# nyu-systems/CLM-GS

Hardware: AMD Instinct MI355X
Metric: training images/s (Rubble-4K 28M Gaussians clm_offload) (higher is better)
Workload: dtype f32

## Files before the change

### clm_gs_amd/csrc/isect3.hip

```cpp
#include <stdlib.h>

#include "common.h"
#include "gs_math.h"
#include "isect_math.h"
#include "radix.h"

namespace clmgs {

constexpr int I3_ROUNDS = 4;
constexpr int I3_CHUNK = 256 * I3_ROUNDS;
constexpr int I3_BIG = 64;
constexpr int I3_SCAN_BLOCKS = 64;

__host__ __device__ static inline int i3_chunks(int V) { return (V + I3_CHUNK - 1) / I3_CHUNK; }

struct RowBox { int x0, y0, bw, nt; unsigned long long mask; };

__device__ __forceinline__ RowBox unpack_row(unsigned long long b, unsigned long long m) {
  RowBox r;
  r.x0 = (int)(b & 0xFFFF); r.y0 = (int)((b >> 16) & 0xFFFF);
  const int x1 = (int)((b >> 32) & 0xFFFF), y1 = (int)(b >> 48);
  r.bw = x1 - r.x0; r.nt = r.bw * (y1 - r.y0);
  r.mask = r.nt > 64 ? ~0ull : (m & (r.nt == 64 ? ~0ull : ((1ull << r.nt) - 1ull)));
  return r;
}

constexpr int I3_WIN = 4096;

struct I3Window { int x0, y0, w, h; bool lds; };

__device__ __forceinline__ I3Window block_window(int x0, int y0, int x1, int y1, int* red ) {
  int v0 = x0, v1 = y0, v2 = -x1, v3 = -y1;
#pragma unroll
  for (int o = 32; o > 0; o >>= 1) {
    v0 = min(v0, __shfl_xor(v0, o, 64)); v1 = min(v1, __shfl_xor(v1, o, 64));
    v2 = min(v2, __shfl_xor(v2, o, 64)); v3 = min(v3, __shfl_xor(v3, o, 64));
  }
  const int wid = threadIdx.x >> 6;
  __syncthreads();
  if ((threadIdx.x & 63) == 0) { red[wid * 4 + 0] = v0; red[wid * 4 + 1] = v1; red[wid * 4 + 2] = v2; red[wid * 4 + 3] = v3; }
  __syncthreads();
  I3Window W;
  W.x0 = min(min(red[0], red[4]), min(red[8], red[12]));
  W.y0 = min(min(red[1], red[5]), min(red[9], red[13]));
  const int X1 = -min(min(red[2], red[6]), min(red[10], red[14]));
  const int Y1 = -min(min(red[3], red[7]), min(red[11], red[15]));
  W.w = max(X1 - W.x0, 0); W.h = max(Y1 - W.y0, 0);
  W.lds = (long long)W.w * W.h <= I3_WIN;
  return W;
}

__global__ void __launch_bounds__(256)
isect3_rows_kernel(int V, const int32_t* __restrict__ radii, const float* __restrict__ means2d,
                   const float4* __restrict__ packed, float tile_size, int tile_w, int tile_h,
                   unsigned long long* __restrict__ box_by_row, uint32_t* __restrict__ tile_cnt,
                   int64_t* __restrict__ row_cum, int64_t* __restrict__ blk_tot, int64_t* __restrict__ blk_ref) {
  __shared__ long long wsum[4];
  __shared__ int big_rows[I3_CHUNK];
  __shared__ int n_big;
  __shared__ unsigned long long rsum[4];
  __shared__ int red[16];
  __shared__ uint32_t win[I3_WIN];
  const int tid = threadIdx.x, chunk = blockIdx.x;
  if (tid == 0) n_big = 0;
  for (int q = tid; q < I3_WIN; q += 256) win[q] = 0u;
  __syncthreads();
  long long c[I3_ROUNDS];
  unsigned long long bx[I3_ROUNDS], mk[I3_ROUNDS];
  unsigned long long ref = 0ull;
  int wx0 = 1 << 30, wy0 = 1 << 30, wx1 = -(1 << 30), wy1 = -(1 << 30);
#pragma unroll
  for (int r = 0; r < I3_ROUNDS; ++r) {
    const int i = chunk * I3_CHUNK + r * 256 + tid;
    c[r] = 0; bx[r] = 0ull; mk[r] = 0ull;
    if (i < V) {
      const int rad = radii[i];
      unsigned long long b = 0ull, m = ~0ull;
      int cnt = 0;
      if (rad > 0) {
        const float2 mm = *reinterpret_cast<const float2*>(means2d + 2 * (size_t)i);
        const TileBox tb = tile_box(mm.x, mm.y, (float)rad, tile_size, tile_w, tile_h);
        b = pack_box(tb);
        if (packed) m = exact_tile_mask(packed + 4 * (size_t)i, tb.x0, tb.y0, tb.x1, tb.y1);
        const RowBox rb = unpack_row(b, m);
        ref += (unsigned long long)rb.nt;
        if (rb.nt > I3_BIG) {
          cnt = rb.nt;
          big_rows[atomicAdd(&n_big, 1)] = i;
        } else {
          cnt = __popcll(rb.mask);
          if (cnt) {
            bx[r] = b; mk[r] = rb.mask;
            wx0 = min(wx0, tb.x0); wy0 = min(wy0, tb.y0); wx1 = max(wx1, tb.x1); wy1 = max(wy1, tb.y1);
          }
        }
      }
      box_by_row[2 * (size_t)i] = cnt > 0 ? b : 0ull;
      box_by_row[2 * (size_t)i + 1] = m;
      c[r] = cnt;
    }
  }
  const I3Window W = block_window(wx0, wy0, wx1, wy1, red);
#pragma unroll
  for (int r = 0; r < I3_ROUNDS; ++r) {
    unsigned long long mm2 = mk[r];
    if (!mm2) continue;
    const RowBox rb = unpack_row(bx[r], mm2);
    while (mm2) {
      const int t = __ffsll((long long)mm2) - 1;
      mm2 &= mm2 - 1ull;
      const int ty = rb.y0 + t / rb.bw, tx = rb.x0 + t % rb.bw;
      if (W.lds) atomicAdd(&win[(ty - W.y0) * W.w + (tx - W.x0)], 1u);
      else atomicAdd(&tile_cnt[ty * tile_w + tx], 1u);
    }
  }
  {
    long long inc[I3_ROUNDS];
    long long carry = 0;
#pragma unroll
    for (int r = 0; r < I3_ROUNDS; ++r) {
      const long long incl = block_incl_scan_i64(c[r], wsum);
      inc[r] = carry + incl;
      carry += wsum[0] + wsum[1] + wsum[2] + wsum[3];
    }
    if (tid == 0) blk_tot[chunk] = carry;
#pragma unroll
    for (int r = 0; r < I3_ROUNDS; ++r) {
      const int i = chunk * I3_CHUNK + r * 256 + tid;
      if (i < V) row_cum[i] = inc[r];
    }
  }
  ref = (unsigned long long)wave_sum_i64((long long)ref);
  __syncthreads();
  if ((tid & 63) == 0) rsum[tid >> 6] = ref;
  if (W.lds) {
    const int nwin = W.w * W.h;
    for (int q = tid; q < nwin; q += 256) {
      const uint32_t v = win[q];
      if (v) atomicAdd(&tile_cnt[(W.y0 + q / W.w) * tile_w + W.x0 + q % W.w], v);
    }
  }
  __syncthreads();
  if (tid == 0) blk_ref[chunk] = (int64_t)(rsum[0] + rsum[1] + rsum[2] + rsum[3]);
  const int nb = n_big;
  for (int q = 0; q < nb; ++q) {
    const int i = big_rows[q];
    const RowBox rb = unpack_row(box_by_row[2 * (size_t)i], ~0ull);
    for (int t = tid; t < rb.nt; t += 256) {
      const int ty = t / rb.bw, tx = t - ty * rb.bw;
      atomicAdd(&tile_cnt[(rb.y0 + ty) * tile_w + rb.x0 + tx], 1u);
    }
  }
}

__global__ void __launch_bounds__(256)
isect3_rows_finish_kernel(int V, int64_t* __restrict__ row_cum, const int64_t* __restrict__ blk_tot,
                          const int64_t* __restrict__ blk_ref, int64_t* __restrict__ totals, int n_tiles,
                          const uint32_t* __restrict__ tile_cnt, int64_t* __restrict__ slice_tot) {
  __shared__ long long wsum[4];
  const int chunk = blockIdx.x, tid = threadIdx.x;
  for (int sl = chunk; sl < I3_SCAN_BLOCKS; sl += gridDim.x) {
    const int per = (n_tiles + I3_SCAN_BLOCKS - 1) / I3_SCAN_BLOCKS;
    const int t_lo = min(n_tiles, sl * per), t_hi = min(n_tiles, t_lo + per);
    long long sum = 0;
    for (int t = t_lo + tid; t < t_hi; t += 256) sum += tile_cnt[t];
    sum = wave_sum_i64(sum);
    __syncthreads();
    if ((tid & 63) == 0) wsum[tid >> 6] = sum;
    __syncthreads();
    if (tid == 0) slice_tot[sl] = wsum[0] + wsum[1] + wsum[2] + wsum[3];
    __syncthreads();
  }
  long long part = 0;
  for (int j = tid; j < chunk; j += 256) part += blk_tot[j];
  part = wave_sum_i64(part);
  if ((tid & 63) == 0) wsum[tid >> 6] = part;
  __syncthreads();
  const long long off = wsum[0] + wsum[1] + wsum[2] + wsum[3];
  if (chunk > 0) {
#pragma unroll
    for (int r = 0; r < I3_ROUNDS; ++r) {
      const int i = chunk * I3_CHUNK + r * 256 + tid;
      if (i < V) row_cum[i] += off;
    }
  }
  if (chunk == (int)gridDim.x - 1) {
    long long ref = 0;
    for (int j = tid; j < (int)gridDim.x; j += 256) ref += blk_ref[j];
    ref = wave_sum_i64(ref);
    __syncthreads();
    if ((tid & 63) == 0) wsum[tid >> 6] = ref;
    __syncthreads();
    if (tid == 0) { totals[0] = off + blk_tot[chunk]; totals[1] = wsum[0] + wsum[1] + wsum[2] + wsum[3]; }
  }
}

__global__ void __launch_bounds__(256)
isect3_tile_scan_kernel(int n_tiles, const uint32_t* __restrict__ tile_cnt, int64_t n, const int64_t* __restrict__ n_dev,
                        int32_t* __restrict__ offsets, uint32_t* __restrict__ cursor, uint32_t* __restrict__ big_count,
                        const int64_t* __restrict__ slice_tot) {
  __shared__ long long wsum[4];
  if (n_dev) n = min(n, *n_dev);
  const int tid = threadIdx.x;
  if (blockIdx.x == 0 && tid == 0) *big_count = 0u;
  const int per = (n_tiles + I3_SCAN_BLOCKS - 1) / I3_SCAN_BLOCKS;
  const int t_lo = min(n_tiles, (int)blockIdx.x * per), t_hi = min(n_tiles, t_lo + per);
  long long carry = 0;
  for (int sl = 0; sl < (int)blockIdx.x; ++sl) carry += slice_tot[sl];
  for (int base = t_lo; base < t_hi; base += 256) {
    const int t = base + tid;
    const uint32_t v = t < t_hi ? tile_cnt[t] : 0u;
    const long long incl = block_incl_scan_i64((long long)v, wsum);
    const long long ex = carry + incl - v;
    if (t < t_hi) {
      offsets[t] = (int32_t)min(ex, (long long)n);
      cursor[t] = (uint32_t)ex;
    }
    carry += wsum[0] + wsum[1] + wsum[2] + wsum[3];
    __syncthreads();
  }
}

struct I3Rec { uint32_t depth; int32_t row; int32_t slot; int32_t pad; };

__global__ void __launch_bounds__(256)
isect3_scatter_kernel(int V, const unsigned long long* __restrict__ box_by_row, const float* __restrict__ depths,
                      const int64_t* __restrict__ row_cum, int tile_w, uint32_t* __restrict__ cursor, int64_t n,
                      const int64_t* __restrict__ n_dev, int4* __restrict__ recs) {
  __shared__ int big_rows[I3_CHUNK];
  __shared__ int n_big;
  __shared__ int red[16];
  __shared__ uint32_t win[I3_WIN];
  if (n_dev) n = min(n, *n_dev);
  const int tid = threadIdx.x, chunk = blockIdx.x;
  if (tid == 0) n_big = 0;
  for (int q = tid; q < I3_WIN; q += 256) win[q] = 0u;
  __syncthreads();
  unsigned long long bx[I3_ROUNDS], mk[I3_ROUNDS];
  int wx0 = 1 << 30, wy0 = 1 << 30, wx1 = -(1 << 30), wy1 = -(1 << 30);
#pragma unroll
  for (int r = 0; r < I3_ROUNDS; ++r) {
    const int i = chunk * I3_CHUNK + r * 256 + tid;
    bx[r] = 0ull; mk[r] = 0ull;
    if (i >= V) continue;
    const unsigned long long b = box_by_row[2 * (size_t)i];
    if (b == 0ull) continue;
    const RowBox rb = unpack_row(b, box_by_row[2 * (size_t)i + 1]);
    if (rb.nt > I3_BIG) { big_rows[atomicAdd(&n_big, 1)] = i; continue; }
    bx[r] = b; mk[r] = rb.mask;
    wx0 = min(wx0, rb.x0); wy0 = min(wy0, rb.y0);
    wx1 = max(wx1, rb.x0 + rb.bw); wy1 = max(wy1, rb.y0 + rb.nt / rb.bw);
  }
  const I3Window W = block_window(wx0, wy0, wx1, wy1, red);
  if (W.lds) {
#pragma unroll
    for (int r = 0; r < I3_ROUNDS; ++r) {
      unsigned long long mm = mk[r];
      if (!mm) continue;
      const RowBox rb = unpack_row(bx[r], mm);
      while (mm) {
        const int t = __ffsll((long long)mm) - 1;
        mm &= mm - 1ull;
        atomicAdd(&win[(rb.y0 + t / rb.bw - W.y0) * W.w + (rb.x0 + t % rb.bw - W.x0)], 1u);
      }
    }
    __syncthreads();
    const int nwin = W.w * W.h;
    for (int q = tid; q < nwin; q += 256) {
      const uint32_t v = win[q];
      if (v) win[q] = atomicAdd(&cursor[(W.y0 + q / W.w) * tile_w + W.x0 + q % W.w], v);
    }
    __syncthreads();
  }
#pragma unroll
  for (int r = 0; r < I3_ROUNDS; ++r) {
    unsigned long long mm = mk[r];
    if (!mm) continue;
    const int i = chunk * I3_CHUNK + r * 256 + tid;
    const RowBox rb = unpack_row(bx[r], mm);
    const uint32_t dk = (uint32_t)__float_as_int(depths[i]);
    int slot = i > 0 ? (int)row_cum[i - 1] : 0;
    while (mm) {
      const int t = __ffsll((long long)mm) - 1;
      mm &= mm - 1ull;
      const int ty = rb.y0 + t / rb.bw, tx = rb.x0 + t % rb.bw;
      const uint32_t pos = W.lds ? atomicAdd(&win[(ty - W.y0) * W.w + (tx - W.x0)], 1u)
                                 : atomicAdd(&cursor[ty * tile_w + tx], 1u);
      if ((int64_t)pos < n) recs[pos] = make_int4((int)dk, i, slot, 0);
      ++slot;
    }
  }
  __syncthreads();
  const int nb = n_big;
  for (int q = 0; q < nb; ++q) {
    const int i = big_rows[q];
    const RowBox rb = unpack_row(box_by_row[2 * (size_t)i], ~0ull);
    const uint32_t dk = (uint32_t)__float_as_int(depths[i]);
    const int slot0 = i > 0 ? (int)row_cum[i - 1] : 0;
    for (int t = tid; t < rb.nt; t += 256) {
      const int ty = t / rb.bw, tx = t - ty * rb.bw;
      const uint32_t pos = atomicAdd(&cursor[(rb.y0 + ty) * tile_w + rb.x0 + tx], 1u);
      if ((int64_t)pos < n) recs[pos] = make_int4((int)dk, i, slot0 + t, 0);
    }
  }
}

template <int THREADS, typename SyncFn>
__device__ __forceinline__ void bitonic_sort_kv(unsigned long long* keys, int32_t* vals, int len, int tid, SyncFn sync) {
  int P = 1;
  while (P < len) P <<= 1;
  for (int k = 2; k <= P; k <<= 1) {
    for (int j = k >> 1; j > 0; j >>= 1) {
      sync();
      for (int c = tid; c < (P >> 1); c += THREADS) {
        const int lo = ((c & ~(j - 1)) << 1) | (c & (j - 1));
        const int hi = (j == (k >> 1)) ? (lo ^ (k - 1)) : (lo | j);
        if (hi < len) {
          const unsigned long long a = keys[lo], b = keys[hi];
          if (b < a) {
            keys[lo] = b; keys[hi] = a;
            const int32_t va = vals[lo], vb = vals[hi];
            vals[lo] = vb; vals[hi] = va;
          }
        }
      }
    }
  }
  sync();
}

constexpr int I3_SMALL = 1024;
constexpr int I3_LDS_BIG = 8192;

__device__ __forceinline__ void i3_write_out(int tile, int s, int len, const unsigned long long* keys, const int32_t* vals,
                                             int tid, int threads, int32_t* __restrict__ flatten_ids,
                                             int32_t* __restrict__ emit_slot, int64_t* __restrict__ isect_ids) {
  for (int q = tid; q < len; q += threads) {
    const unsigned long long k = keys[q];
    flatten_ids[s + q] = (int32_t)(k & 0xFFFFFFFFull);
    if (emit_slot) emit_slot[s + q] = vals[q];
    if (isect_ids) isect_ids[s + q] = ((int64_t)tile << 32) | (int64_t)(k >> 32);
  }
}

template <int LO, int CAP>
__global__ void __launch_bounds__(64)
isect3_sort_small_kernel(int n_tiles, const int32_t* __restrict__ offsets, int64_t n, const int64_t* __restrict__ n_dev,
                         const int4* __restrict__ recs, int32_t* __restrict__ flatten_ids,
                         int32_t* __restrict__ emit_slot, int64_t* __restrict__ isect_ids,
                         uint32_t* __restrict__ big_count, int32_t* __restrict__ big_list) {
  __shared__ unsigned long long keys[CAP];
  __shared__ int32_t vals[CAP];
  if (n_dev) n = min(n, *n_dev);
  const int tile = (int)xcd_remap(blockIdx.x, (unsigned)n_tiles);
  const int tid = threadIdx.x;
  const int s = offsets[tile];
  const int e = (tile == n_tiles - 1) ? (int)n : offsets[tile + 1];
  const int len = e - s;
  if (CAP == I3_SMALL && len > I3_SMALL && tid == 0) big_list[atomicAdd(big_count, 1u)] = tile;
  if (len <= LO || len > CAP) return;
  for (int q = tid; q < len; q += 64) {
    const int4 r = recs[s + q];
    keys[q] = ((unsigned long long)(uint32_t)r.x << 32) | (unsigned long long)(uint32_t)r.y;
    vals[q] = r.z;
  }
  bitonic_sort_kv<64>(keys, vals, len, tid, [] { __syncthreads(); });
  i3_write_out(tile, s, len, keys, vals, tid, 64, flatten_ids, emit_slot, isect_ids);
}

template <int E>
__device__ __forceinline__ void rank_sort_tile(unsigned long long* keys, int tile, int s, int len, int tid,
                                               const int4* __restrict__ recs, int32_t* __restrict__ flatten_ids,
                                               int32_t* __restrict__ emit_slot, int64_t* __restrict__ isect_ids) {
  unsigned long long key[E];
  int32_t slot[E];
#pragma unroll
  for (int r = 0; r < E; ++r) {
    const int q = tid + 64 * r;
    key[r] = ~0ull; slot[r] = 0;
    if (q < len) {
      const int4 rc = recs[s + q];
      key[r] = ((unsigned long long)(uint32_t)rc.x << 32) | (unsigned long long)(uint32_t)rc.y;
      slot[r] = rc.z;
      keys[q] = key[r];
    }
  }
  __syncthreads();
  int cnt[E];
#pragma unroll
  for (int r = 0; r < E; ++r) cnt[r] = 0;
  int j = 0;
  for (; j + 4 <= len; j += 4) {
    const unsigned long long k0 = keys[j], k1 = keys[j + 1], k2 = keys[j + 2], k3 = keys[j + 3];
#pragma unroll
    for (int r = 0; r < E; ++r)
      cnt[r] += (int)(k0 < key[r]) + (int)(k1 < key[r]) + (int)(k2 < key[r]) + (int)(k3 < key[r]);
  }
  for (; j < len; ++j) {
    const unsigned long long k0 = keys[j];
#pragma unroll
    for (int r = 0; r < E; ++r) cnt[r] += (int)(k0 < key[r]);
  }
#pragma unroll
  for (int r = 0; r < E; ++r) {
    if (tid + 64 * r < len) {
      const int o = s + cnt[r];
      flatten_ids[o] = (int32_t)(key[r] & 0xFFFFFFFFull);
      if (emit_slot) emit_slot[o] = slot[r];
      if (isect_ids) isect_ids[o] = ((int64_t)tile << 32) | (int64_t)(key[r] >> 32);
    }
  }
}

__global__ void __launch_bounds__(64)
isect3_sort_rank_kernel(int n_tiles, const int32_t* __restrict__ offsets, int64_t n, const int64_t* __restrict__ n_dev,
                        const int4* __restrict__ recs, int32_t* __restrict__ flatten_ids,
                        int32_t* __restrict__ emit_slot, int64_t* __restrict__ isect_ids) {
  constexpr int CAP = 256;
  __shared__ unsigned long long keys[CAP];
  if (n_dev) n = min(n, *n_dev);
  const int tile = (int)xcd_remap(blockIdx.x, (unsigned)n_tiles);
  const int tid = threadIdx.x;
  const int s = offsets[tile];
  const int e = (tile == n_tiles - 1) ? (int)n : offsets[tile + 1];
  const int len = e - s;
  if (len <= 0 || len > CAP) return;
  if (len <= 64) rank_sort_tile<1>(keys, tile, s, len, tid, recs, flatten_ids, emit_slot, isect_ids);
  else if (len <= 128) rank_sort_tile<2>(keys, tile, s, len, tid, recs, flatten_ids, emit_slot, isect_ids);
  else if (len <= 192) rank_sort_tile<3>(keys, tile, s, len, tid, recs, flatten_ids, emit_slot, isect_ids);
  else rank_sort_tile<4>(keys, tile, s, len, tid, recs, flatten_ids, emit_slot, isect_ids);
}

__global__ void __launch_bounds__(256)
isect3_sort_big_kernel(int n_tiles, const int32_t* __restrict__ offsets, int64_t n, const int64_t* __restrict__ n_dev,
                       const int4* __restrict__ recs, unsigned long long* __restrict__ gkeys, int32_t* __restrict__ gvals,
                       int32_t* __restrict__ flatten_ids, int32_t* __restrict__ emit_slot,
                       int64_t* __restrict__ isect_ids, const uint32_t* __restrict__ big_count,
                       const int32_t* __restrict__ big_list) {
  extern __shared__ __attribute__((aligned(16))) unsigned char dyn[];
  if (n_dev) n = min(n, *n_dev);
  const int tid = threadIdx.x;
  const int n_big = (int)*big_count;
  for (int w = blockIdx.x; w < n_big; w += gridDim.x) {
    const int tile = big_list[w];
    const int s = offsets[tile];
    const int e = (tile == n_tiles - 1) ? (int)n : offsets[tile + 1];
    const int len = e - s;
    __syncthreads();
    unsigned long long* keys;
    int32_t* vals;
    if (len <= I3_LDS_BIG) {
      keys = reinterpret_cast<unsigned long long*>(dyn);
      vals = reinterpret_cast<int32_t*>(dyn + sizeof(unsigned long long) * I3_LDS_BIG);
    } else {
      keys = gkeys + s;
      vals = gvals + s;
    }
    for (int q = tid; q < len; q += 256) {
      const int4 r = recs[s + q];
      keys[q] = ((unsigned long long)(uint32_t)r.x << 32) | (unsigned long long)(uint32_t)r.y;
      vals[q] = r.z;
    }
    bitonic_sort_kv<256>(keys, vals, len, tid, [] { __threadfence_block(); __syncthreads(); });
    i3_write_out(tile, s, len, keys, vals, tid, 256, flatten_ids, emit_slot, isect_ids);
  }
}

}

using namespace clmgs;

static inline size_t i3_front_layout(int V, int n_tiles, size_t* o_cnt, size_t* o_tot, size_t* o_ref) {
  size_t o = align_up((size_t)V * 16, 256);
  *o_cnt = o; o += align_up((size_t)n_tiles * 4, 256) + align_up((size_t)I3_SCAN_BLOCKS * 8, 256);
  *o_tot = o; o += align_up((size_t)i3_chunks(V) * 8, 256);
  *o_ref = o; o += align_up((size_t)i3_chunks(V) * 8, 256);
  return o + 256;
}

extern "C" size_t clmgs_isect3_front_temp_bytes(int V, int n_tiles) {
  if (V <= 0) return 256;
  size_t a, b, c;
  return i3_front_layout(V, n_tiles, &a, &b, &c);
}

extern "C" int clmgs_isect3_front(void* stream, int V, const float* means2d, const int32_t* radii, int tile_size,
                                  int tile_width, int tile_height, const void* packed, int64_t* totals,
                                  int64_t* row_cum, void* temp, size_t temp_bytes) {
  CLMGS_CHECK_ARG(V >= 0 && tile_size > 0 && tile_width > 0 && tile_height > 0);
  CLMGS_CHECK_ARG(tile_width < 65536 && tile_height < 65536 && (int64_t)tile_width * tile_height < ((int64_t)1 << 31));
  if (V == 0) return 0;
  const int n_tiles = tile_width * tile_height;
  CLMGS_CHECK_ARG(means2d && radii && totals && row_cum && temp);
  CLMGS_CHECK_ARG(!packed || tile_size == 16);
  CLMGS_CHECK_ARG(temp_bytes >= clmgs_isect3_front_temp_bytes(V, n_tiles));
  hipStream_t s = (hipStream_t)stream;
  size_t o_cnt, o_tot, o_ref;
  i3_front_layout(V, n_tiles, &o_cnt, &o_tot, &o_ref);
  char* base = (char*)temp;
  unsigned long long* box_by_row = (unsigned long long*)base;
  uint32_t* tile_cnt = (uint32_t*)(base + o_cnt);
  int64_t* blk_tot = (int64_t*)(base + o_tot);
  int64_t* blk_ref = (int64_t*)(base + o_ref);
  CLMGS_HIP(hipMemsetAsync(tile_cnt, 0, (size_t)n_tiles * 4, s));
  const int nck = i3_chunks(V);
  hipLaunchKernelGGL(isect3_rows_kernel, dim3(nck), dim3(256), 0, s, V, radii, means2d, (const float4*)packed,
                     (float)tile_size, tile_width, tile_height, box_by_row, tile_cnt, row_cum, blk_tot, blk_ref);
  int64_t* slice_tot = (int64_t*)(base + o_cnt + align_up((size_t)n_tiles * 4, 256));
  hipLaunchKernelGGL(isect3_rows_finish_kernel, dim3(nck), dim3(256), 0, s, V, row_cum, blk_tot, blk_ref, totals, n_tiles,
                     (const uint32_t*)tile_cnt, slice_tot);
  CLMGS_LAUNCH_CHECK();
  return 0;
}

static inline size_t i3_bin_layout(int64_t n, int n_tiles, size_t* o_cur, size_t* o_keys, size_t* o_vals) {
  size_t o = align_up((size_t)n * 16, 256);
  *o_cur = o; o += 2 * align_up((size_t)n_tiles * 4, 256) + 256;
  *o_keys = o; o += align_up((size_t)n * 8, 256);
  *o_vals = o; o += align_up((size_t)n * 4, 256);
  return o + 256;
}

extern "C" size_t clmgs_isect3_bin_temp_bytes(int64_t n_isects, int n_tiles) {
  if (n_isects <= 0) return 256;
  size_t a, b, c;
  return i3_bin_layout(n_isects, n_tiles, &a, &b, &c);
}

static int isect3_bin_impl(void* stream, int V, int64_t n_isects, const int64_t* n_dev, const float* depths,
                           int tile_width, int tile_height, const int64_t* row_cum, const void* front_temp,
                           int32_t* flatten_ids, int32_t* offsets, int64_t* isect_ids, int32_t* emit_slot, void* temp,
                           size_t temp_bytes) {
  CLMGS_CHECK_ARG(V >= 0 && n_isects >= 0 && offsets && tile_width > 0 && tile_height > 0);
  hipStream_t s = (hipStream_t)stream;
  const int n_tiles = tile_width * tile_height;
  if (n_isects == 0 || V == 0) {
    CLMGS_HIP(hipMemsetAsync(offsets, 0, sizeof(int32_t) * (size_t)n_tiles, s));
    return 0;
  }
  CLMGS_CHECK_ARG(n_isects < ((int64_t)1 << 31));
  CLMGS_CHECK_ARG(depths && row_cum && front_temp && flatten_ids && temp);
  CLMGS_CHECK_ARG(temp_bytes >= clmgs_isect3_bin_temp_bytes(n_isects, n_tiles));
  size_t f_cnt, f_tot, f_ref;
  i3_front_layout(V, n_tiles, &f_cnt, &f_tot, &f_ref);
  const unsigned long long* box_by_row = (const unsigned long long*)front_temp;
  const uint32_t* tile_cnt = (const uint32_t*)((const char*)front_temp + f_cnt);
  size_t o_cur, o_keys, o_vals;
  i3_bin_layout(n_isects, n_tiles, &o_cur, &o_keys, &o_vals);
  char* base = (char*)temp;
  int4* recs = (int4*)base;
  uint32_t* cursor = (uint32_t*)(base + o_cur);
  unsigned long long* gkeys = (unsigned long long*)(base + o_keys);
  int32_t* gvals = (int32_t*)(base + o_vals);
  int32_t* big_list = (int32_t*)(base + o_cur + align_up((size_t)n_tiles * 4, 256));
  uint32_t* big_count = (uint32_t*)(base + o_cur + 2 * align_up((size_t)n_tiles * 4, 256));
  const int64_t* slice_tot = (const int64_t*)((const char*)front_temp + f_cnt + align_up((size_t)n_tiles * 4, 256));
  hipLaunchKernelGGL(isect3_tile_scan_kernel, dim3(I3_SCAN_BLOCKS), dim3(256), 0, s, n_tiles, tile_cnt, n_isects, n_dev,
                     offsets, cursor, big_count, slice_tot);
  hipLaunchKernelGGL(isect3_scatter_kernel, dim3(i3_chunks(V)), dim3(256), 0, s, V, box_by_row, depths, row_cum,
                     tile_width, cursor, n_isects, n_dev, recs);
  hipLaunchKernelGGL(isect3_sort_rank_kernel, dim3(n_tiles), dim3(64), 0, s, n_tiles, (const int32_t*)offsets, n_isects,
                     n_dev, (const int4*)recs, flatten_ids, emit_slot, isect_ids);
  hipLaunchKernelGGL((isect3_sort_small_kernel<256, 512>), dim3(n_tiles), dim3(64), 0, s, n_tiles, (const int32_t*)offsets,
                     n_isects, n_dev, (const int4*)recs, flatten_ids, emit_slot, isect_ids, big_count, big_list);
  hipLaunchKernelGGL((isect3_sort_small_kernel<512, I3_SMALL>), dim3(n_tiles), dim3(64), 0, s, n_tiles,
                     (const int32_t*)offsets, n_isects, n_dev, (const int4*)recs, flatten_ids, emit_slot, isect_ids,
                     big_count, big_list);
  static bool lds_set = false;
  const size_t big_lds = (size_t)I3_LDS_BIG * 12;
  if (!lds_set) {
    CLMGS_HIP(hipFuncSetAttribute((const void*)isect3_sort_big_kernel, hipFuncAttributeMaxDynamicSharedMemorySize,
                                  (int)big_lds));
    lds_set = true;
  }
  hipLaunchKernelGGL(isect3_sort_big_kernel, dim3(min(n_tiles, 256)), dim3(256), big_lds, s, n_tiles,
                     (const int32_t*)offsets, n_isects, n_dev, (const int4*)recs, gkeys, gvals, flatten_ids, emit_slot,
                     isect_ids, (const uint32_t*)big_count, (const int32_t*)big_list);
  CLMGS_LAUNCH_CHECK();
  return 0;
}

extern "C" int clmgs_isect3_bin(void* stream, int V, int64_t n_isects, const float* depths, int tile_width,
                                int tile_height, const int64_t* row_cum, const void* front_temp, int32_t* flatten_ids,
                                int32_t* offsets, int64_t* isect_ids, int32_t* emit_slot, void* temp, size_t temp_bytes) {
  return isect3_bin_impl(stream, V, n_isects, nullptr, depths, tile_width, tile_height, row_cum, front_temp, flatten_ids,
                         offsets, isect_ids, emit_slot, temp, temp_bytes);
}

extern "C" int clmgs_isect3_bin_dev(void* stream, int V, int64_t capacity, const int64_t* n_isects_dev,
                                    const float* depths, int tile_width, int tile_height, const int64_t* row_cum,
                                    const void* front_temp, int32_t* flatten_ids, int32_t* offsets, int64_t* isect_ids,
                                    int32_t* emit_slot, void* temp, size_t temp_bytes) {
  CLMGS_CHECK_ARG(n_isects_dev && capacity > 0);
  return isect3_bin_impl(stream, V, capacity, n_isects_dev, depths, tile_width, tile_height, row_cum, front_temp,
                         flatten_ids, offsets, isect_ids, emit_slot, temp, temp_bytes);
}
```

Measured before the change: 206.2.

## Restructure tile-intersection pipeline into single-wave blocks with hierarchical scans and tile lists

Rewrites the intersection row, finish, tile-scan and scatter kernels to use 64-thread single-wave blocks. Block-level scans and window reductions become wave shuffles, and LDS windows are processed per group of four rows. Prefix offsets now use per-superchunk atomically accumulated totals, so each chunk no longer sums all earlier chunk totals. The rank sort kernel now builds per-size-class tile lists so that the medium and large sorts launch compact grids instead of one block per tile. The cost is more global atomics for group totals and big-row handling, and smaller LDS windows that may fall back to global atomics more often.

New measurement: 202.3. 1.9% lower.

```diff
diff --git a/clm_gs_amd/csrc/isect3.hip b/clm_gs_amd/csrc/isect3.hip
--- a/clm_gs_amd/csrc/isect3.hip
+++ b/clm_gs_amd/csrc/isect3.hip
@@ -7,10 +7,13 @@
 
 namespace clmgs {
 
-constexpr int I3_ROUNDS = 4;
-constexpr int I3_CHUNK = 256 * I3_ROUNDS;
+constexpr int I3_ROUNDS = 16;
+constexpr int I3_CHUNK = 64 * I3_ROUNDS;
+constexpr int I3_GROUP = 4;
 constexpr int I3_BIG = 64;
-constexpr int I3_SCAN_BLOCKS = 64;
+constexpr int I3_SCAN_BLOCKS = 256;
+constexpr int I3_SUPER = 64;
+constexpr int I3_LIST_GRID = 1024;
 
 __host__ __device__ static inline int i3_chunks(int V) { return (V + I3_CHUNK - 1) / I3_CHUNK; }
 
@@ -25,282 +28,262 @@
   return r;
 }
 
-constexpr int I3_WIN = 4096;
+constexpr int I3_WIN = 896;
 
 struct I3Window { int x0, y0, w, h; bool lds; };
 
-__device__ __forceinline__ I3Window block_window(int x0, int y0, int x1, int y1, int* red ) {
+__device__ __forceinline__ I3Window wave_window(int x0, int y0, int x1, int y1) {
   int v0 = x0, v1 = y0, v2 = -x1, v3 = -y1;
 #pragma unroll
   for (int o = 32; o > 0; o >>= 1) {
     v0 = min(v0, __shfl_xor(v0, o, 64)); v1 = min(v1, __shfl_xor(v1, o, 64));
     v2 = min(v2, __shfl_xor(v2, o, 64)); v3 = min(v3, __shfl_xor(v3, o, 64));
   }
-  const int wid = threadIdx.x >> 6;
-  __syncthreads();
-  if ((threadIdx.x & 63) == 0) { red[wid * 4 + 0] = v0; red[wid * 4 + 1] = v1; red[wid * 4 + 2] = v2; red[wid * 4 + 3] = v3; }
-  __syncthreads();
   I3Window W;
-  W.x0 = min(min(red[0], red[4]), min(red[8], red[12]));
-  W.y0 = min(min(red[1], red[5]), min(red[9], red[13]));
-  const int X1 = -min(min(red[2], red[6]), min(red[10], red[14]));
-  const int Y1 = -min(min(red[3], red[7]), min(red[11], red[15]));
-  W.w = max(X1 - W.x0, 0); W.h = max(Y1 - W.y0, 0);
+  W.x0 = v0; W.y0 = v1;
+  W.w = max(-v2 - v0, 0); W.h = max(-v3 - v1, 0);
   W.lds = (long long)W.w * W.h <= I3_WIN;
   return W;
 }
 
-__global__ void __launch_bounds__(256)
+__global__ void __launch_bounds__(64)
 isect3_rows_kernel(int V, const int32_t* __restrict__ radii, const float* __restrict__ means2d,
                    const float4* __restrict__ packed, float tile_size, int tile_w, int tile_h,
                    unsigned long long* __restrict__ box_by_row, uint32_t* __restrict__ tile_cnt,
-                   int64_t* __restrict__ row_cum, int64_t* __restrict__ blk_tot, int64_t* __restrict__ blk_ref) {
-  __shared__ long long wsum[4];
-  __shared__ int big_rows[I3_CHUNK];
-  __shared__ int n_big;
-  __shared__ unsigned long long rsum[4];
-  __shared__ int red[16];
+                   int64_t* __restrict__ row_cum, int64_t* __restrict__ blk_tot, unsigned long long* __restrict__ grp) {
   __shared__ uint32_t win[I3_WIN];
-  const int tid = threadIdx.x, chunk = blockIdx.x;
-  if (tid == 0) n_big = 0;
-  for (int q = tid; q < I3_WIN; q += 256) win[q] = 0u;
-  __syncthreads();
-  long long c[I3_ROUNDS];
-  unsigned long long bx[I3_ROUNDS], mk[I3_ROUNDS];
+  const int lane = threadIdx.x, chunk = blockIdx.x;
+  long long carry = 0;
   unsigned long long ref = 0ull;
-  int wx0 = 1 << 30, wy0 = 1 << 30, wx1 = -(1 << 30), wy1 = -(1 << 30);
-#pragma unroll
-  for (int r = 0; r < I3_ROUNDS; ++r) {
-    const int i = chunk * I3_CHUNK + r * 256 + tid;
-    c[r] = 0; bx[r] = 0ull; mk[r] = 0ull;
-    if (i < V) {
-      const int rad = radii[i];
-      unsigned long long b = 0ull, m = ~0ull;
-      int cnt = 0;
-      if (rad > 0) {
-        const float2 mm = *reinterpret_cast<const float2*>(means2d + 2 * (size_t)i);
-        const TileBox tb = tile_box(mm.x, mm.y, (float)rad, tile_size, tile_w, tile_h);
-        b = pack_box(tb);
-        if (packed) m = exact_tile_mask(packed + 4 * (size_t)i, tb.x0, tb.y0, tb.x1, tb.y1);
-        const RowBox rb = unpack_row(b, m);
-        ref += (unsigned long long)rb.nt;
-        if (rb.nt > I3_BIG) {
-          cnt = rb.nt;
-          big_rows[atomicAdd(&n_big, 1)] = i;
-        } else {
-          cnt = __popcll(rb.mask);
-          if (cnt) {
-            bx[r] = b; mk[r] = rb.mask;
-            wx0 = min(wx0, tb.x0); wy0 = min(wy0, tb.y0); wx1 = max(wx1, tb.x1); wy1 = max(wy1, tb.y1);
+  for (int g = 0; g < I3_ROUNDS / I3_GROUP; ++g) {
+    const int base = chunk * I3_CHUNK + g * I3_GROUP * 64;
+    if (base >= V) break;
+    unsigned long long bx[I3_GROUP], mk[I3_GROUP];
+    int wx0 = 1 << 30, wy0 = 1 << 30, wx1 = -(1 << 30), wy1 = -(1 << 30);
+#pragma unroll
+    for (int r = 0; r < I3_GROUP; ++r) {
+      const int i = base + r * 64 + lane;
+      bx[r] = 0ull; mk[r] = 0ull;
+      long long cnt = 0;
+      if (i < V) {
+        const int rad = radii[i];
+        unsigned long long b = 0ull, m = ~0ull;
+        if (rad > 0) {
+          const float2 mm = *reinterpret_cast<const float2*>(means2d + 2 * (size_t)i);
+          const TileBox tb = tile_box(mm.x, mm.y, (float)rad, tile_size, tile_w, tile_h);
+          b = pack_box(tb);
+          if (packed) m = exact_tile_mask(packed + 4 * (size_t)i, tb.x0, tb.y0, tb.x1, tb.y1);
+          const RowBox rb = unpack_row(b, m);
+          ref += (unsigned long long)rb.nt;
+          if (rb.nt > I3_BIG) {
+            cnt = rb.nt;
+            bx[r] = b; mk[r] = ~0ull;
+          } else {
+            cnt = __popcll(rb.mask);
+            if (cnt) {
+              bx[r] = b; mk[r] = rb.mask;
+              wx0 = min(wx0, tb.x0); wy0 = min(wy0, tb.y0); wx1 = max(wx1, tb.x1); wy1 = max(wy1, tb.y1);
+            }
           }
         }
-      }
-      box_by_row[2 * (size_t)i] = cnt > 0 ? b : 0ull;
-      box_by_row[2 * (size_t)i + 1] = m;
-      c[r] = cnt;
-    }
-  }
-  const I3Window W = block_window(wx0, wy0, wx1, wy1, red);
-#pragma unroll
-  for (int r = 0; r < I3_ROUNDS; ++r) {
-    unsigned long long mm2 = mk[r];
-    if (!mm2) continue;
-    const RowBox rb = unpack_row(bx[r], mm2);
-    while (mm2) {
-      const int t = __ffsll((long long)mm2) - 1;
-      mm2 &= mm2 - 1ull;
-      const int ty = rb.y0 + t / rb.bw, tx = rb.x0 + t % rb.bw;
-      if (W.lds) atomicAdd(&win[(ty - W.y0) * W.w + (tx - W.x0)], 1u);
-      else atomicAdd(&tile_cnt[ty * tile_w + tx], 1u);
-    }
-  }
-  {
-    long long inc[I3_ROUNDS];
-    long long carry = 0;
-#pragma unroll
-    for (int r = 0; r < I3_ROUNDS; ++r) {
-      const long long incl = block_incl_scan_i64(c[r], wsum);
-      inc[r] = carry + incl;
-      carry += wsum[0] + wsum[1] + wsum[2] + wsum[3];
-    }
-    if (tid == 0) blk_tot[chunk] = carry;
-#pragma unroll
-    for (int r = 0; r < I3_ROUNDS; ++r) {
-      const int i = chunk * I3_CHUNK + r * 256 + tid;
-      if (i < V) row_cum[i] = inc[r];
+        box_by_row[2 * (size_t)i] = cnt > 0 ? b : 0ull;
+        box_by_row[2 * (size_t)i + 1] = m;
+      }
+      const long long incl = wave_incl_scan_i64(cnt, lane);
+      if (i < V) row_cum[i] = carry + incl;
+      carry += __shfl(incl, 63, 64);
+    }
+    const I3Window W = wave_window(wx0, wy0, wx1, wy1);
+    const int nwin = W.w * W.h;
+    if (W.lds)
+      for (int q = lane; q < nwin; q += 64) win[q] = 0u;
+    __syncthreads();
+#pragma unroll
+    for (int r = 0; r < I3_GROUP; ++r) {
+      unsigned long long mm2 = mk[r];
+      const RowBox rb = unpack_row(bx[r], mm2);
+      if (rb.nt > I3_BIG) continue;
+      while (mm2) {
+        const int t = __ffsll((long long)mm2) - 1;
+        mm2 &= mm2 - 1ull;
+        const int ty = rb.y0 + t / rb.bw, tx = rb.x0 + t % rb.bw;
+        if (W.lds) atomicAdd(&win[(ty - W.y0) * W.w + (tx - W.x0)], 1u);
+        else atomicAdd(&tile_cnt[ty * tile_w + tx], 1u);
+      }
+    }
+    __syncthreads();
+    if (W.lds) {
+      for (int q = lane; q < nwin; q += 64) {
+        const uint32_t v = win[q];
+        if (v) atomicAdd(&tile_cnt[(W.y0 + q / W.w) * tile_w + W.x0 + q % W.w], v);
+      }
+    }
+    __syncthreads();
+#pragma unroll
+    for (int r = 0; r < I3_GROUP; ++r) {
+      unsigned long long bigs = __ballot(unpack_row(bx[r], mk[r]).nt > I3_BIG);
+      while (bigs) {
+        const int src = __ffsll((long long)bigs) - 1;
+        bigs &= bigs - 1ull;
+        const RowBox rb = unpack_row(__shfl(bx[r], src, 64), ~0ull);
+        for (int t = lane; t < rb.nt; t += 64) {
+          const int ty = t / rb.bw, tx = t - ty * rb.bw;
+          atomicAdd(&tile_cnt[(rb.y0 + ty) * tile_w + rb.x0 + tx], 1u);
+        }
+      }
     }
   }
   ref = (unsigned long long)wave_sum_i64((long long)ref);
-  __syncthreads();
-  if ((tid & 63) == 0) rsum[tid >> 6] = ref;
-  if (W.lds) {
-    const int nwin = W.w * W.h;
-    for (int q = tid; q < nwin; q += 256) {
-      const uint32_t v = win[q];
-      if (v) atomicAdd(&tile_cnt[(W.y0 + q / W.w) * tile_w + W.x0 + q % W.w], v);
-    }
-  }
-  __syncthreads();
-  if (tid == 0) blk_ref[chunk] = (int64_t)(rsum[0] + rsum[1] + rsum[2] + rsum[3]);
-  const int nb = n_big;
-  for (int q = 0; q < nb; ++q) {
-    const int i = big_rows[q];
-    const RowBox rb = unpack_row(box_by_row[2 * (size_t)i], ~0ull);
-    for (int t = tid; t < rb.nt; t += 256) {
-      const int ty = t / rb.bw, tx = t - ty * rb.bw;
-      atomicAdd(&tile_cnt[(rb.y0 + ty) * tile_w + rb.x0 + tx], 1u);
-    }
-  }
-}
-
-__global__ void __launch_bounds__(256)
+  if (lane == 0) {
+    blk_tot[chunk] = carry;
+    atomicAdd(&grp[2 * (chunk / I3_SUPER)], (unsigned long long)carry);
+    atomicAdd(&grp[2 * (chunk / I3_SUPER) + 1], ref);
+  }
+}
+
+__global__ void __launch_bounds__(64)
 isect3_rows_finish_kernel(int V, int64_t* __restrict__ row_cum, const int64_t* __restrict__ blk_tot,
-                          const int64_t* __restrict__ blk_ref, int64_t* __restrict__ totals, int n_tiles,
+                          const unsigned long long* __restrict__ grp, int64_t* __restrict__ totals, int n_tiles,
                           const uint32_t* __restrict__ tile_cnt, int64_t* __restrict__ slice_tot) {
-  __shared__ long long wsum[4];
-  const int chunk = blockIdx.x, tid = threadIdx.x;
+  const int chunk = blockIdx.x, lane = threadIdx.x;
   for (int sl = chunk; sl < I3_SCAN_BLOCKS; sl += gridDim.x) {
     const int per = (n_tiles + I3_SCAN_BLOCKS - 1) / I3_SCAN_BLOCKS;
     const int t_lo = min(n_tiles, sl * per), t_hi = min(n_tiles, t_lo + per);
     long long sum = 0;
-    for (int t = t_lo + tid; t < t_hi; t += 256) sum += tile_cnt[t];
+    for (int t = t_lo + lane; t < t_hi; t += 64) sum += tile_cnt[t];
     sum = wave_sum_i64(sum);
-    __syncthreads();
-    if ((tid & 63) == 0) wsum[tid >> 6] = sum;
-    __syncthreads();
-    if (tid == 0) slice_tot[sl] = wsum[0] + wsum[1] + wsum[2] + wsum[3];
-    __syncthreads();
-  }
+    if (lane == 0) slice_tot[sl] = sum;
+  }
+  const int g0 = chunk / I3_SUPER;
   long long part = 0;
-  for (int j = tid; j < chunk; j += 256) part += blk_tot[j];
-  part = wave_sum_i64(part);
-  if ((tid & 63) == 0) wsum[tid >> 6] = part;
-  __syncthreads();
-  const long long off = wsum[0] + wsum[1] + wsum[2] + wsum[3];
+  for (int j = lane; j < g0; j += 64) part += (long long)grp[2 * j];
+  if (g0 * I3_SUPER + lane < chunk) part += blk_tot[g0 * I3_SUPER + lane];
+  const long long off = wave_sum_i64(part);
   if (chunk > 0) {
-#pragma unroll
+#pragma unroll 4
     for (int r = 0; r < I3_ROUNDS; ++r) {
-      const int i = chunk * I3_CHUNK + r * 256 + tid;
+      const int i = chunk * I3_CHUNK + r * 64 + lane;
       if (i < V) row_cum[i] += off;
     }
   }
   if (chunk == (int)gridDim.x - 1) {
     long long ref = 0;
-    for (int j = tid; j < (int)gridDim.x; j += 256) ref += blk_ref[j];
+    for (int j = lane; j <= g0; j += 64) ref += (long long)grp[2 * j + 1];
     ref = wave_sum_i64(ref);
-    __syncthreads();
-    if ((tid & 63) == 0) wsum[tid >> 6] = ref;
-    __syncthreads();
-    if (tid == 0) { totals[0] = off + blk_tot[chunk]; totals[1] = wsum[0] + wsum[1] + wsum[2] + wsum[3]; }
-  }
-}
-
-__global__ void __launch_bounds__(256)
+    if (lane == 0) { totals[0] = off + blk_tot[chunk]; totals[1] = ref; }
+  }
+}
+
+__global__ void __launch_bounds__(64)
 isect3_tile_scan_kernel(int n_tiles, const uint32_t* __restrict__ tile_cnt, int64_t n, const int64_t* __restrict__ n_dev,
-                        int32_t* __restrict__ offsets, uint32_t* __restrict__ cursor, uint32_t* __restrict__ big_count,
+                        int32_t* __restrict__ offsets, uint32_t* __restrict__ cursor, uint32_t* __restrict__ list_count,
                         const int64_t* __restrict__ slice_tot) {
-  __shared__ long long wsum[4];
   if (n_dev) n = min(n, *n_dev);
-  const int tid = threadIdx.x;
-  if (blockIdx.x == 0 && tid == 0) *big_count = 0u;
+  const int lane = threadIdx.x;
+  if (blockIdx.x == 0 && lane < 3) list_count[lane] = 0u;
   const int per = (n_tiles + I3_SCAN_BLOCKS - 1) / I3_SCAN_BLOCKS;
   const int t_lo = min(n_tiles, (int)blockIdx.x * per), t_hi = min(n_tiles, t_lo + per);
-  long long carry = 0;
-  for (int sl = 0; sl < (int)blockIdx.x; ++sl) carry += slice_tot[sl];
-  for (int base = t_lo; base < t_hi; base += 256) {
-    const int t = base + tid;
+  long long part = 0;
+  for (int sl = lane; sl < (int)blockIdx.x; sl += 64) part += slice_tot[sl];
+  long long carry = wave_sum_i64(part);
+  for (int base = t_lo; base < t_hi; base += 64) {
+    const int t = base + lane;
     const uint32_t v = t < t_hi ? tile_cnt[t] : 0u;
-    const long long incl = block_incl_scan_i64((long long)v, wsum);
+    const long long incl = wave_incl_scan_i64((long long)v, lane);
     const long long ex = carry + incl - v;
     if (t < t_hi) {
       offsets[t] = (int32_t)min(ex, (long long)n);
       cursor[t] = (uint32_t)ex;
     }
-    carry += wsum[0] + wsum[1] + wsum[2] + wsum[3];
-    __syncthreads();
+    carry += __shfl(incl, 63, 64);
   }
 }
 
 struct I3Rec { uint32_t depth; int32_t row; int32_t slot; int32_t pad; };
 
-__global__ void __launch_bounds__(256)
+__global__ void __launch_bounds__(64)
 isect3_scatter_kernel(int V, const unsigned long long* __restrict__ box_by_row, const float* __restrict__ depths,
                       const int64_t* __restrict__ row_cum, int tile_w, uint32_t* __restrict__ cursor, int64_t n,
                       const int64_t* __restrict__ n_dev, int4* __restrict__ recs) {
-  __shared__ int big_rows[I3_CHUNK];
-  __shared__ int n_big;
-  __shared__ int red[16];
   __shared__ uint32_t win[I3_WIN];
   if (n_dev) n = min(n, *n_dev);
-  const int tid = threadIdx.x, chunk = blockIdx.x;
-  if (tid == 0) n_big = 0;
-  for (int q = tid; q < I3_WIN; q += 256) win[q] = 0u;
-  __syncthreads();
-  unsigned long long bx[I3_ROUNDS], mk[I3_ROUNDS];
-  int wx0 = 1 << 30, wy0 = 1 << 30, wx1 = -(1 << 30), wy1 = -(1 << 30);
-#pragma unroll
-  for (int r = 0; r < I3_ROUNDS; ++r) {
-    const int i = chunk * I3_CHUNK + r * 256 + tid;
-    bx[r] = 0ull; mk[r] = 0ull;
-    if (i >= V) continue;
-    const unsigned long long b = box_by_row[2 * (size_t)i];
-    if (b == 0ull) continue;
-    const RowBox rb = unpack_row(b, box_by_row[2 * (size_t)i + 1]);
-    if (rb.nt > I3_BIG) { big_rows[atomicAdd(&n_big, 1)] = i; continue; }
-    bx[r] = b; mk[r] = rb.mask;
-    wx0 = min(wx0, rb.x0); wy0 = min(wy0, rb.y0);
-    wx1 = max(wx1, rb.x0 + rb.bw); wy1 = max(wy1, rb.y0 + rb.nt / rb.bw);
-  }
-  const I3Window W = block_window(wx0, wy0, wx1, wy1, red);
-  if (W.lds) {
-#pragma unroll
-    for (int r = 0; r < I3_ROUNDS; ++r) {
+  const int lane = threadIdx.x, chunk = blockIdx.x;
+  for (int g = 0; g < I3_ROUNDS / I3_GROUP; ++g) {
+    const int base = chunk * I3_CHUNK + g * I3_GROUP * 64;
+    if (base >= V) break;
+    unsigned long long bx[I3_GROUP], mk[I3_GROUP];
+    int wx0 = 1 << 30, wy0 = 1 << 30, wx1 = -(1 << 30), wy1 = -(1 << 30);
+#pragma unroll
+    for (int r = 0; r < I3_GROUP; ++r) {
+      const int i = base + r * 64 + lane;
+      bx[r] = 0ull; mk[r] = 0ull;
+      if (i >= V) continue;
+      const unsigned long long b = box_by_row[2 * (size_t)i];
+      if (b == 0ull) continue;
+      const RowBox rb = unpack_row(b, box_by_row[2 * (size_t)i + 1]);
+      bx[r] = b; mk[r] = rb.mask;
+      if (rb.nt > I3_BIG) continue;
+      wx0 = min(wx0, rb.x0); wy0 = min(wy0, rb.y0);
+      wx1 = max(wx1, rb.x0 + rb.bw); wy1 = max(wy1, rb.y0 + rb.nt / rb.bw);
+    }
+    const I3Window W = wave_window(wx0, wy0, wx1, wy1);
+    if (W.lds) {
+      const int nwin = W.w * W.h;
+      for (int q = lane; q < nwin; q += 64) win[q] = 0u;
+      __syncthreads();
+#pragma unroll
+      for (int r = 0; r < I3_GROUP; ++r) {
+        unsigned long long mm = mk[r];
+        const RowBox rb = unpack_row(bx[r], mm);
+        if (rb.nt > I3_BIG) continue;
+        while (mm) {
+          const int t = __ffsll((long long)mm) - 1;
+          mm &= mm - 1ull;
+          atomicAdd(&win[(rb.y0 + t / rb.bw - W.y0) * W.w + (rb.x0 + t % rb.bw - W.x0)], 1u);
+        }
+      }
+      __syncthreads();
+      for (int q = lane; q < nwin; q += 64) {
+        const uint32_t v = win[q];
+        if (v) win[q] = atomicAdd(&cursor[(W.y0 + q / W.w) * tile_w + W.x0 + q % W.w], v);
+      }
+      __syncthreads();
+    }
+#pragma unroll
+    for (int r = 0; r < I3_GROUP; ++r) {
       unsigned long long mm = mk[r];
-      if (!mm) continue;
       const RowBox rb = unpack_row(bx[r], mm);
+      if (rb.nt > I3_BIG || !mm) continue;
+      const int i = base + r * 64 + lane;
+      const uint32_t dk = (uint32_t)__float_as_int(depths[i]);
+      int slot = i > 0 ? (int)row_cum[i - 1] : 0;
       while (mm) {
         const int t = __ffsll((long long)mm) - 1;
         mm &= mm - 1ull;
-        atomicAdd(&win[(rb.y0 + t / rb.bw - W.y0) * W.w + (rb.x0 + t % rb.bw - W.x0)], 1u);
+        const int ty = rb.y0 + t / rb.bw, tx = rb.x0 + t % rb.bw;
+        const uint32_t pos = W.lds ? atomicAdd(&win[(ty - W.y0) * W.w + (tx - W.x0)], 1u)
+                                   : atomicAdd(&cursor[ty * tile_w + tx], 1u);
+        if ((int64_t)pos < n) recs[pos] = make_int4((int)dk, i, slot, 0);
+        ++slot;
       }
     }
     __syncthreads();
-    const int nwin = W.w * W.h;
-    for (int q = tid; q < nwin; q += 256) {
-      const uint32_t v = win[q];
-      if (v) win[q] = atomicAdd(&cursor[(W.y0 + q / W.w) * tile_w + W.x0 + q % W.w], v);
-    }
-    __syncthreads();
-  }
-#pragma unroll
-  for (int r = 0; r < I3_ROUNDS; ++r) {
-    unsigned long long mm = mk[r];
-    if (!mm) continue;
-    const int i = chunk * I3_CHUNK + r * 256 + tid;
-    const RowBox rb = unpack_row(bx[r], mm);
-    const uint32_t dk = (uint32_t)__float_as_int(depths[i]);
-    int slot = i > 0 ? (int)row_cum[i - 1] : 0;
-    while (mm) {
-      const int t = __ffsll((long long)mm) - 1;
-      mm &= mm - 1ull;
-      const int ty = rb.y0 + t / rb.bw, tx = rb.x0 + t % rb.bw;
-      const uint32_t pos = W.lds ? atomicAdd(&win[(ty - W.y0) * W.w + (tx - W.x0)], 1u)
-                                 : atomicAdd(&cursor[ty * tile_w + tx], 1u);
-      if ((int64_t)pos < n) recs[pos] = make_int4((int)dk, i, slot, 0);
-      ++slot;
-    }
-  }
-  __syncthreads();
-  const int nb = n_big;
-  for (int q = 0; q < nb; ++q) {
-    const int i = big_rows[q];
-    const RowBox rb = unpack_row(box_by_row[2 * (size_t)i], ~0ull);
-    const uint32_t dk = (uint32_t)__float_as_int(depths[i]);
-    const int slot0 = i > 0 ? (int)row_cum[i - 1] : 0;
-    for (int t = tid; t < rb.nt; t += 256) {
-      const int ty = t / rb.bw, tx = t - ty * rb.bw;
-      const uint32_t pos = atomicAdd(&cursor[(rb.y0 + ty) * tile_w + rb.x0 + tx], 1u);
-      if ((int64_t)pos < n) recs[pos] = make_int4((int)dk, i, slot0 + t, 0);
+#pragma unroll
+    for (int r = 0; r < I3_GROUP; ++r) {
+      unsigned long long bigs = __ballot(unpack_row(bx[r], mk[r]).nt > I3_BIG);
+      while (bigs) {
+        const int src = __ffsll((long long)bigs) - 1;
+        bigs &= bigs - 1ull;
+        const int i = base + r * 64 + src;
+        const RowBox rb = unpack_row(__shfl(bx[r], src, 64), ~0ull);
+        const uint32_t dk = (uint32_t)__float_as_int(depths[i]);
+        const int slot0 = i > 0 ? (int)row_cum[i - 1] : 0;
+        for (int t = lane; t < rb.nt; t += 64) {
+          const int ty = t / rb.bw, tx = t - ty * rb.bw;
+          const uint32_t pos = atomicAdd(&cursor[(rb.y0 + ty) * tile_w + rb.x0 + tx], 1u);
+          if ((int64_t)pos < n) recs[pos] = make_int4((int)dk, i, slot0 + t, 0);
+        }
+      }
     }
   }
 }
@@ -343,29 +326,33 @@
   }
 }
 
-template <int LO, int CAP>
+__device__ __forceinline__ int i3_list_class(int len) { return len <= 512 ? 0 : (len <= I3_SMALL ? 1 : 2); }
+
+template <int CAP>
 __global__ void __launch_bounds__(64)
 isect3_sort_small_kernel(int n_tiles, const int32_t* __restrict__ offsets, int64_t n, const int64_t* __restrict__ n_dev,
                          const int4* __restrict__ recs, int32_t* __restrict__ flatten_ids,
                          int32_t* __restrict__ emit_slot, int64_t* __restrict__ isect_ids,
-                         uint32_t* __restrict__ big_count, int32_t* __restrict__ big_list) {
+                         const uint32_t* __restrict__ list_count, const int32_t* __restrict__ list) {
   __shared__ unsigned long long keys[CAP];
   __shared__ int32_t vals[CAP];
   if (n_dev) n = min(n, *n_dev);
-  const int tile = (int)xcd_remap(blockIdx.x, (unsigned)n_tiles);
   const int tid = threadIdx.x;
-  const int s = offsets[tile];
-  const int e = (tile == n_tiles - 1) ? (int)n : offsets[tile + 1];
-  const int len = e - s;
-  if (CAP == I3_SMALL && len > I3_SMALL && tid == 0) big_list[atomicAdd(big_count, 1u)] = tile;
-  if (len <= LO || len > CAP) return;
-  for (int q = tid; q < len; q += 64) {
-    const int4 r = recs[s + q];
-    keys[q] = ((unsigned long long)(uint32_t)r.x << 32) | (unsigned long long)(uint32_t)r.y;
-    vals[q] = r.z;
-  }
-  bitonic_sort_kv<64>(keys, vals, len, tid, [] { __syncthreads(); });
-  i3_write_out(tile, s, len, keys, vals, tid, 64, flatten_ids, emit_slot, isect_ids);
+  const int n_list = (int)*list_count;
+  for (int w = blockIdx.x; w < n_list; w += gridDim.x) {
+    const int tile = list[w];
+    const int s = offsets[tile];
+    const int e = (tile == n_tiles - 1) ? (int)n : offsets[tile + 1];
+    const int len = min(e - s, CAP);
+    __syncthreads();
+    for (int q = tid; q < len; q += 64) {
+      const int4 r = recs[s + q];
+      keys[q] = ((unsigned long long)(uint32_t)r.x << 32) | (unsigned long long)(uint32_t)r.y;
+      vals[q] = r.z;
+    }
+    bitonic_sort_kv<64>(keys, vals, len, tid, [] { __syncthreads(); });
+    i3_write_out(tile, s, len, keys, vals, tid, 64, flatten_ids, emit_slot, isect_ids);
+  }
 }
 
 template <int E>
@@ -415,7 +402,8 @@
 __global__ void __launch_bounds__(64)
 isect3_sort_rank_kernel(int n_tiles, const int32_t* __restrict__ offsets, int64_t n, const int64_t* __restrict__ n_dev,
                         const int4* __restrict__ recs, int32_t* __restrict__ flatten_ids,
-                        int32_t* __restrict__ emit_slot, int64_t* __restrict__ isect_ids) {
+                        int32_t* __restrict__ emit_slot, int64_t* __restrict__ isect_ids,
+                        uint32_t* __restrict__ list_count, int32_t* __restrict__ lists) {
   constexpr int CAP = 256;
   __shared__ unsigned long long keys[CAP];
   if (n_dev) n = min(n, *n_dev);
@@ -424,7 +412,12 @@
   const int s = offsets[tile];
   const int e = (tile == n_tiles - 1) ? (int)n : offsets[tile + 1];
   const int len = e - s;
-  if (len <= 0 || len > CAP) return;
+  if (len > CAP) {
+    const int c = i3_list_class(len);
+    if (tid == 0) lists[(size_t)c * n_tiles + atomicAdd(&list_count[c], 1u)] = tile;
+    return;
+  }
+  if (len <= 0) return;
   if (len <= 64) rank_sort_tile<1>(keys, tile, s, len, tid, recs, flatten_ids, emit_slot, isect_ids);
   else if (len <= 128) rank_sort_tile<2>(keys, tile, s, len, tid, recs, flatten_ids, emit_slot, isect_ids);
   else if (len <= 192) rank_sort_tile<3>(keys, tile, s, len, tid, recs, flatten_ids, emit_slot, isect_ids);
@@ -470,18 +463,24 @@
 
 using namespace clmgs;
 
-static inline size_t i3_front_layout(int V, int n_tiles, size_t* o_cnt, size_t* o_tot, size_t* o_ref) {
+struct I3Front { size_t cnt, grp, zero_bytes, slice, tot, bytes; };
+
+static inline I3Front i3_front_layout(int V, int n_tiles) {
+  I3Front f;
+  const size_t n_grp = ((size_t)i3_chunks(V) + I3_SUPER - 1) / I3_SUPER;
   size_t o = align_up((size_t)V * 16, 256);
-  *o_cnt = o; o += align_up((size_t)n_tiles * 4, 256) + align_up((size_t)I3_SCAN_BLOCKS * 8, 256);
-  *o_tot = o; o += align_up((size_t)i3_chunks(V) * 8, 256);
-  *o_ref = o; o += align_up((size_t)i3_chunks(V) * 8, 256);
-  return o + 256;
+  f.cnt = o; o += align_up((size_t)n_tiles * 4, 256);
+  f.grp = o; o += align_up(n_grp * 16, 256);
+  f.zero_bytes = o - f.cnt;
+  f.slice = o; o += align_up((size_t)I3_SCAN_BLOCKS * 8, 256);
+  f.tot = o; o += align_up((size_t)i3_chunks(V) * 8, 256);
+  f.bytes = o + 256;
+  return f;
 }
 
 extern "C" size_t clmgs_isect3_front_temp_bytes(int V, int n_tiles) {
   if (V <= 0) return 256;
-  size_t a, b, c;
-  return i3_front_layout(V, n_tiles, &a, &b, &c);
+  return i3_front_layout(V, n_tiles).bytes;
 }
 
 extern "C" int clmgs_isect3_front(void* stream, int V, const float* means2d, const int32_t* radii, int tile_size,
@@ -495,27 +494,26 @@
   CLMGS_CHECK_ARG(!packed || tile_size == 16);
   CLMGS_CHECK_ARG(temp_bytes >= clmgs_isect3_front_temp_bytes(V, n_tiles));
   hipStream_t s = (hipStream_t)stream;
-  size_t o_cnt, o_tot, o_ref;
-  i3_front_layout(V, n_tiles, &o_cnt, &o_tot, &o_ref);
+  const I3Front f = i3_front_layout(V, n_tiles);
   char* base = (char*)temp;
   unsigned long long* box_by_row = (unsigned long long*)base;
-  uint32_t* tile_cnt = (uint32_t*)(base + o_cnt);
-  int64_t* blk_tot = (int64_t*)(base + o_tot);
-  int64_t* blk_ref = (int64_t*)(base + o_ref);
-  CLMGS_HIP(hipMemsetAsync(tile_cnt, 0, (size_t)n_tiles * 4, s));
+  uint32_t* tile_cnt = (uint32_t*)(base + f.cnt);
+  unsigned long long* grp = (unsigned long long*)(base + f.grp);
+  int64_t* slice_tot = (int64_t*)(base + f.slice);
+  int64_t* blk_tot = (int64_t*)(base + f.tot);
+  CLMGS_HIP(hipMemsetAsync(tile_cnt, 0, f.zero_bytes, s));
   const int nck = i3_chunks(V);
-  hipLaunchKernelGGL(isect3_rows_kernel, dim3(nck), dim3(256), 0, s, V, radii, means2d, (const float4*)packed,
-                     (float)tile_size, tile_width, tile_height, box_by_row, tile_cnt, row_cum, blk_tot, blk_ref);
-  int64_t* slice_tot = (int64_t*)(base + o_cnt + align_up((size_t)n_tiles * 4, 256));
-  hipLaunchKernelGGL(isect3_rows_finish_kernel, dim3(nck), dim3(256), 0, s, V, row_cum, blk_tot, blk_ref, totals, n_tiles,
-                     (const uint32_t*)tile_cnt, slice_tot);
+  hipLaunchKernelGGL(isect3_rows_kernel, dim3(nck), dim3(64), 0, s, V, radii, means2d, (const float4*)packed,
+                     (float)tile_size, tile_width, tile_height, box_by_row, tile_cnt, row_cum, blk_tot, grp);
+  hipLaunchKernelGGL(isect3_rows_finish_kernel, dim3(nck), dim3(64), 0, s, V, row_cum, (const int64_t*)blk_tot,
+                     (const unsigned long long*)grp, totals, n_tiles, (const uint32_t*)tile_cnt, slice_tot);
   CLMGS_LAUNCH_CHECK();
   return 0;
 }
 
 static inline size_t i3_bin_layout(int64_t n, int n_tiles, size_t* o_cur, size_t* o_keys, size_t* o_vals) {
   size_t o = align_up((size_t)n * 16, 256);
-  *o_cur = o; o += 2 * align_up((size_t)n_tiles * 4, 256) + 256;
+  *o_cur = o; o += align_up((size_t)n_tiles * 4, 256) + align_up((size_t)n_tiles * 12, 256) + 256;
   *o_keys = o; o += align_up((size_t)n * 8, 256);
   *o_vals = o; o += align_up((size_t)n * 4, 256);
   return o + 256;
@@ -541,10 +539,9 @@
   CLMGS_CHECK_ARG(n_isects < ((int64_t)1 << 31));
   CLMGS_CHECK_ARG(depths && row_cum && front_temp && flatten_ids && temp);
   CLMGS_CHECK_ARG(temp_bytes >= clmgs_isect3_bin_temp_bytes(n_isects, n_tiles));
-  size_t f_cnt, f_tot, f_ref;
-  i3_front_layout(V, n_tiles, &f_cnt, &f_tot, &f_ref);
+  const I3Front f = i3_front_layout(V, n_tiles);
   const unsigned long long* box_by_row = (const unsigned long long*)front_temp;
-  const uint32_t* tile_cnt = (const uint32_t*)((const char*)front_temp + f_cnt);
+  const uint32_t* tile_cnt = (const uint32_t*)((const char*)front_temp + f.cnt);
   size_t o_cur, o_keys, o_vals;
   i3_bin_layout(n_isects, n_tiles, &o_cur, &o_keys, &o_vals);
   char* base = (char*)temp;
@@ -552,20 +549,24 @@
   uint32_t* cursor = (uint32_t*)(base + o_cur);
   unsigned long long* gkeys = (unsigned long long*)(base + o_keys);
   int32_t* gvals = (int32_t*)(base + o_vals);
-  int32_t* big_list = (int32_t*)(base + o_cur + align_up((size_t)n_tiles * 4, 256));
-  uint32_t* big_count = (uint32_t*)(base + o_cur + 2 * align_up((size_t)n_tiles * 4, 256));
-  const int64_t* slice_tot = (const int64_t*)((const char*)front_temp + f_cnt + align_up((size_t)n_tiles * 4, 256));
-  hipLaunchKernelGGL(isect3_tile_scan_kernel, dim3(I3_SCAN_BLOCKS), dim3(256), 0, s, n_tiles, tile_cnt, n_isects, n_dev,
-                     offsets, cursor, big_count, slice_tot);
-  hipLaunchKernelGGL(isect3_scatter_kernel, dim3(i3_chunks(V)), dim3(256), 0, s, V, box_by_row, depths, row_cum,
+  int32_t* lists = (int32_t*)(base + o_cur + align_up((size_t)n_tiles * 4, 256));
+  uint32_t* list_count = (uint32_t*)(base + o_cur + align_up((size_t)n_tiles * 4, 256) + align_up((size_t)n_tiles * 12, 256));
+  const int64_t* slice_tot = (const int64_t*)((const char*)front_temp + f.slice);
+  hipLaunchKernelGGL(isect3_tile_scan_kernel, dim3(I3_SCAN_BLOCKS), dim3(64), 0, s, n_tiles, tile_cnt, n_isects, n_dev,
+                     offsets, cursor, list_count, slice_tot);
+  hipLaunchKernelGGL(isect3_scatter_kernel, dim3(i3_chunks(V)), dim3(64), 0, s, V, box_by_row, depths, row_cum,
                      tile_width, cursor, n_isects, n_dev, recs);
   hipLaunchKernelGGL(isect3_sort_rank_kernel, dim3(n_tiles), dim3(64), 0, s, n_tiles, (const int32_t*)offsets, n_isects,
-                     n_dev, (const int4*)recs, flatten_ids, emit_slot, isect_ids);
-  hipLaunchKernelGGL((isect3_sort_small_kernel<256, 512>), dim3(n_tiles), dim3(64), 0, s, n_tiles, (const int32_t*)offsets,
-                     n_isects, n_dev, (const int4*)recs, flatten_ids, emit_slot, isect_ids, big_count, big_list);
-  hipLaunchKernelGGL((isect3_sort_small_kernel<512, I3_SMALL>), dim3(n_tiles), dim3(64), 0, s, n_tiles,
+                     n_dev, (const int4*)recs, flatten_ids, emit_slot, isect_ids, list_count, lists);
+  const int list_grid = min(n_tiles, I3_LIST_GRID);
+  hipLaunchKernelGGL((isect3_sort_small_kernel<512>), dim3(list_grid), dim3(64), 0, s, n_tiles, (const int32_t*)offsets,
+                     n_isects, n_dev, (const int4*)recs, flatten_ids, emit_slot, isect_ids,
+                     (const uint32_t*)list_count, (const int32_t*)lists);
+  hipLaunchKernelGGL((isect3_sort_small_kernel<I3_SMALL>), dim3(list_grid), dim3(64), 0, s, n_tiles,
                      (const int32_t*)offsets, n_isects, n_dev, (const int4*)recs, flatten_ids, emit_slot, isect_ids,
-                     big_count, big_list);
+                     (const uint32_t*)(list_count + 1), (const int32_t*)(lists + n_tiles));
+  const uint32_t* big_count = list_count + 2;
+  const int32_t* big_list = lists + 2 * (size_t)n_tiles;
   static bool lds_set = false;
   const size_t big_lds = (size_t)I3_LDS_BIG * 12;
   if (!lds_set) {
@@ -575,7 +576,7 @@
   }
   hipLaunchKernelGGL(isect3_sort_big_kernel, dim3(min(n_tiles, 256)), dim3(256), big_lds, s, n_tiles,
                      (const int32_t*)offsets, n_isects, n_dev, (const int4*)recs, gkeys, gvals, flatten_ids, emit_slot,
-                     isect_ids, (const uint32_t*)big_count, (const int32_t*)big_list);
+                     isect_ids, big_count, big_list);
   CLMGS_LAUNCH_CHECK();
   return 0;
 }
```
